# AlexandreGac/alphazero-chess

Hardware: AMD Instinct MI355X
Metric: MCTS sims/sec at 800 sims/move, 20x256 net; self-play games/hr at 1/2/4/8 GPU (higher is better)
Workload: dtype f32

## Files before the change

alphazero-chess_amd/azchess/_lib.py:

```python
import ctypes as C
import os

import numpy as np

_HERE = os.path.dirname(os.path.abspath(__file__))
LIB_PATH = os.environ.get("AZ_LIB") or os.path.join(_HERE, "libaz.so")
CSRC = os.path.join(os.path.dirname(_HERE), "csrc")

ACTION_SPACE = 4096
MAX_MOVES = 256
ONGOING, DRAW, WHITE_WINS, BLACK_WINS, ILLEGAL = 0, 1, 2, 3, -1
DTYPE_F32, DTYPE_BF16, DTYPE_FP8 = 0, 1, 2
EVAL_NET, EVAL_SYNTHETIC, EVAL_CALLBACK = 0, 1, 2
PACKED_KINDS = ("conv_w", "conv_b", "in_pk32", "wino_w", "wino16_w", "wino16_us", "w8", "w8s", "b8", "head",
                "head_frag", "head_frag32")


class AzPos(C.Structure):
    _fields_ = [("bb", C.c_uint64 * 8), ("turn", C.c_uint8), ("castling", C.c_uint8), ("ep", C.c_uint8),
                ("flags", C.c_uint8), ("halfmoves", C.c_uint16), ("fullmoves", C.c_uint16),
                ("rep_key", C.c_uint64)]


POS_DTYPE = np.dtype({
# ... 51 lines not shown
ALLREDUCE_FN = C.CFUNCTYPE(C.c_int, C.c_void_p, C.POINTER(C.c_float), C.c_size_t)

P = C.POINTER
SIGNATURES = [
    ("az_last_error", C.c_char_p, []),
    ("az_version", C.c_int, []),
    ("az_device_count", C.c_int, [P(C.c_int)]),
    ("az_device_synchronize", C.c_int, [C.c_int]),
    ("az_pos_startpos", C.c_int, [P(AzPos)]),
    ("az_pos_from_fen", C.c_int, [C.c_char_p, P(AzPos)]),
    ("az_pos_to_fen", C.c_int, [P(AzPos), C.c_char_p, C.c_int]),
    ("az_pos_fen_key", C.c_uint64, [P(AzPos)]),
    ("az_pos_legal_indices", C.c_int, [P(AzPos), P(C.c_int32), C.c_int]),
    ("az_pos_play_index", C.c_int, [P(AzPos), C.c_int32, P(AzPos)]),
    ("az_move_to_index", C.c_int, [C.c_int, C.c_int, C.c_int]),
    ("az_pos_outcome", C.c_int, [P(AzPos)]),
    ("az_pos_encode", C.c_int, [P(AzPos), P(C.c_float)]),
    ("az_game_create", C.c_int, [P(C.c_void_p)]),
    ("az_game_clone", C.c_int, [C.c_void_p, P(C.c_void_p)]),
    ("az_game_destroy", C.c_int, [C.c_void_p]),
    ("az_game_position", C.c_int, [C.c_void_p, P(AzPos)]),
    ("az_game_history", C.c_int, [C.c_void_p, P(C.c_int32), C.c_int]),
    ("az_game_play", C.c_int, [C.c_void_p, C.c_int32]),
    ("az_net_num_params", C.c_size_t, [C.c_int, C.c_int]),
    ("az_net_create", C.c_int, [P(AzNetDesc), P(C.c_float), C.c_size_t, C.c_int, P(C.c_void_p)]),
    ("az_net_destroy", C.c_int, [C.c_void_p]),
    ("az_net_tower_kernel", C.c_int, [C.c_void_p, C.c_char_p, C.c_int]),
    ("az_net_wino_streamed_points", C.c_int, [C.c_void_p]),
    ("az_net_wino_accumulators", C.c_int, [C.c_void_p]),
    ("az_net_wino_v_rows", C.c_int, [C.c_void_p]),
    ("az_wino_vrows_layout", C.c_int, [C.c_void_p] * 5),
    ("az_net_wino_boards", C.c_int, [C.c_void_p]),
    ("az_wino_boards_layout", C.c_int, [C.c_void_p] * 6),
    ("az_wino16_pack", C.c_int, [P(C.c_float), C.c_int, C.c_int, P(C.c_uint16), C.c_size_t, P(C.c_float)]),
    ("az_wino16_pack_rows", C.c_int, [P(C.c_float), C.c_int, P(C.c_uint16), C.c_size_t, P(C.c_float)]),
    ("az_net_load_mpk",C.c_int, [C.c_char_p, C.c_int, C.c_int, P(C.c_float), C.c_size_t]),
    ("az_net_save_mpk", C.c_int, [C.c_char_p, C.c_int, C.c_int, P(C.c_float), C.c_size_t]),
    ("az_net_forward", C.c_int, [C.c_void_p, P(C.c_float), C.c_int, P(C.c_float), P(C.c_float)]),
    ("az_net_forward_device", C.c_int, [C.c_void_p, C.c_void_p, C.c_int, C.c_void_p, C.c_void_p, C.c_void_p]),
    ("az_net_update_device", C.c_int, [C.c_void_p, C.c_void_p, C.c_size_t, C.c_void_p]),
    ("az_net_update", C.c_int, [C.c_void_p, P(C.c_float), C.c_size_t]),
    ("az_net_update_from_trainer", C.c_int, [C.c_void_p, C.c_void_p]),
    ("az_net_generation", C.c_int64, [C.c_void_p]),
    ("az_net_get_weights", C.c_int, [C.c_void_p, P(C.c_float), C.c_size_t]),
    ("az_net_packed_read", C.c_int, [C.c_void_p, C.c_int, C.c_int, C.c_void_p, C.c_size_t]),
    ("az_search_default_cfg", C.c_int, [P(AzSearchCfg)]),
    ("az_search_create", C.c_int, [C.c_void_p, P(AzSearchCfg), C.c_int, P(C.c_void_p)]),
    ("az_search_destroy", C.c_int, [C.c_void_p]),
    ("az_search_set_evaluator", C.c_int, [C.c_void_p, C.c_void_p, C.c_void_p]),
    ("az_search_set_roots", C.c_int, [C.c_void_p, P(C.c_int32), P(C.c_int32), P(C.c_int32), P(C.c_int32),
                                      C.c_int]),
    ("az_search_set_roots_from", C.c_int, [C.c_void_p, P(AzPos), P(C.c_int32), P(C.c_int32), P(C.c_int32),
                                           P(C.c_int32), C.c_int]),
    ("az_search_run", C.c_int, [C.c_void_p, P(C.c_float), P(C.c_uint32), P(C.c_int32)]),
    ("az_search_read_roots", C.c_int, [C.c_void_p, P(C.c_float), P(C.c_uint32), P(C.c_int32)]),
    ("az_search_advance", C.c_int, [C.c_void_p, P(C.c_int32), C.c_int, P(C.c_int32)]),
    ("az_selfplay_reset", C.c_int, [C.c_void_p]),
    ("az_selfplay_step", C.c_int, [C.c_void_p, P(C.c_int), P(C.c_int)]),
    ("az_selfplay_run_sims", C.c_int, [C.c_void_p, C.c_int, P(C.c_int), P(C.c_int), P(C.c_int)]),
    ("az_selfplay_drain", C.c_int, [C.c_void_p, P(AzEpisodeStep), C.c_int]),
    ("az_selfplay_adopt_net", C.c_int, [C.c_void_p]),
    ("az_search_adopt_net", C.c_int, [C.c_void_p, C.c_int]),
    ("az_selfplay_inflight", C.c_int, [C.c_void_p, P(C.c_int32), P(C.c_int32), P(C.c_int32), P(C.c_int32),
                                       P(C.c_int32), C.c_int]),
    ("az_search_stats_get", C.c_int, [C.c_void_p, P(AzSearchStats)]),
    ("az_search_persistent", C.c_int, [C.c_void_p]),
# ... 130 lines not shown
```

alphazero-chess_amd/azchess/agent.py:

```python
import ctypes as C
import os

import numpy as np

from . import _lib as L
from .parameters import NUM_FILTERS, NUM_RES_BLOCKS, SEED


def num_params(blocks, filters):
    return int(L.lib.az_net_num_params(int(blocks), int(filters)))


def param_shapes(blocks, filters):
    F = filters
    out = [("input_conv.weight", (F, 19, 3, 3), 19 * 9), ("input_conv.bias", (F,), 19 * 9),
           ("input_bn", (4, F), None)]
    for b in range(blocks):
        for k in (1, 2):
            out += [("res_blocks.%d.conv%d.weight" % (b, k), (F, F, 3, 3), F * 9),
                    ("res_blocks.%d.conv%d.bias" % (b, k), (F,), F * 9),
                    ("res_blocks.%d.bn%d" % (b, k), (4, F), None)]
    out += [("policy_conv_1.weight", (32, F, 1, 1), F), ("policy_conv_1.bias", (32,), F), ("policy_bn", (4, 32), None),
            ("policy_conv_2.weight", (64, 32, 1, 1), 32), ("policy_conv_2.bias", (64,), 32),
            ("value_conv.weight", (8, F, 1, 1), F), ("value_conv.bias", (8,), F), ("value_bn", (4, 8), None),
# ... 113 lines not shown
    @property
    def winograd(self):
        return "Winograd" in self.tower_kernel

    def __del__(self):
        try:
            L.lib.az_net_destroy(self._h)
        except Exception:
            pass

    def save_file(self, path):
        save_mpk(path, self.weights, self.blocks, self.filters)

    def forward(self, x):
        x = np.ascontiguousarray(x, np.float32).reshape(-1, 19 * 64)
        n = x.shape[0]
        pol = np.zeros((n, 4096), np.float32)
        val = np.zeros(n, np.float32)
        L.check(L.lib.az_net_forward(self._h, L.fptr(x), n, L.fptr(pol), L.fptr(val)))
        return pol, val


def wino_vrows_layout():
    t = dict(write=np.empty((16, 64, 4), np.int32), read=np.empty((2, 4, 4, 64), np.int32),
             act=np.empty((16, 64, 4), np.int32), item=np.empty((2, 8, 4), np.int32), dims=np.empty(4, np.int32))
    L.check(L.lib.az_wino_vrows_layout(*(t[k].ctypes.data_as(C.c_void_p) for k in ("write", "read", "act", "item", "dims"))))
    return t


def wino_boards_layout():
    t = dict(item=np.empty((8, 8, 2), np.int32), act=np.empty((2, 2), np.int32), out=np.empty((8, 64, 2, 4), np.int32),
             vbuf=np.empty((2, 2), np.int32), zero=np.empty(64, np.int32), dims=np.empty(8, np.int32))
    L.check(L.lib.az_wino_boards_layout(*(t[k].ctypes.data_as(C.c_void_p) for k in ("item", "act", "out", "vbuf", "zero", "dims"))))
    return t


def mx8_quantize(x):
    x = np.ascontiguousarray(x, np.float32)
    if x.size % 32:
        raise ValueError("mx8_quantize: %d values are not whole blocks of 32" % x.size)
    codes = np.empty(x.shape, np.uint8)
    scales = np.empty(x.size // 32, np.uint8)
    u8 = lambda a: a.ctypes.data_as(L.P(C.c_uint8))
    L.check(L.lib.az_mx8_quantize(L.fptr(x), x.size // 32, u8(codes), u8(scales)))
    return codes, scales


def mx8_conv_probe(filters, act_codes, act_scales, w_codes, w_scales, bias, residual=None, device=0):
    F = int(filters)
    a = np.ascontiguousarray(act_codes, np.uint8)
    n = a.size // (64 * F)
    s = np.ascontiguousarray(act_scales, np.uint8)
    wc, wsc = np.ascontiguousarray(w_codes, np.uint8), np.ascontiguousarray(w_scales, np.uint8)
    b = np.ascontiguousarray(bias, np.float32)
    if a.size != n * 64 * F or s.size != n * 64 * F // 32 or wc.size != F * F * 9 or wsc.size != F * 9 * F // 32 or b.size != F:
        raise ValueError("mx8_conv_probe: operand shapes do not match filters = %d" % F)
    r = None if residual is None else np.ascontiguousarray(residual, np.uint16)
    if r is not None and r.size != a.size:
        raise ValueError("mx8_conv_probe: residual shape")
    out = dict(acc=np.empty((n, 64, F), np.float32), codes=np.empty((n, 64, F), np.uint8),
               scales=np.empty((n, 64, F // 32), np.uint8))
    if r is not None:
        out["bf16"] = np.empty((n, 64, F), np.uint16)
    u8 = lambda x: x.ctypes.data_as(L.P(C.c_uint8))
    u16 = lambda x: None if x is None else x.ctypes.data_as(L.P(C.c_uint16))
    L.check(L.lib.az_mx8_conv_probe(int(device), F, n, u8(a), u8(s), u8(wc), u8(wsc), u16(r), L.fptr(b), L.fptr(out["acc"]),
# ... 3 lines not shown
```

alphazero-chess_amd/csrc/tower.hip:

```cpp
#include <math.h>
#include <stdio.h>
#include <stdlib.h>
#include <string.h>

#include "az_internal.h"
#include "search_dev.h"
#include "wino.h"

#include "tower_dev.h"

namespace azi {

template <int F, bool SEARCH>
__device__ __forceinline__ void tower_board(const __bf16* __restrict__ planes, const TowerArgs& ta, int row0, int nb,
                                            float* __restrict__ pol_out, float* __restrict__ val_out,
                                            const SearchOut& so, int tid) {
    constexpr int BPB = TowerCfg<F>::BPB, WB = TowerCfg<F>::WB, BPW = BPB / WB, NCO = TowerCfg<F>::NCO;
    constexpr int NCW = F / (16 * NCO);
    constexpr int NT = NCW * WB * 64;
    constexpr int RSF = F / 8 + 2, RSI = 32 / 8 + 2;
    constexpr int XSZ = BPB * 64 * RSF;
    constexpr int ZN = 16 + F / 8;
    constexpr int HSZ0 = (HeadsScratch<HeadsCfg<F>::NB, NT>::FLOATS * 4 + 15) / 16;
    constexpr int HSZ = ((XSZ > HSZ0 ? XSZ : HSZ0) + 15) / 16 * 16;
// ... 491 lines not shown
                                        : n * 1024 + wino_toff<F>(0, i * XS + rx);
                    wring[i][rx][n] = __builtin_bit_cast(f32x4, __builtin_amdgcn_raw_buffer_load_b128(r, voff + off, 0, 0));
                }
    }
    for (int b = 0; b < ta.blocks; b++) {
        const unsigned wb3 = b + 1 < ta.blocks ? ta.wwbytes[2 * b + 2] : 0u;
        const __amdgpu_buffer_rsrc_t r1 = t32_rsrc(ta.ww[2 * b], ta.wwbytes[2 * b]);
        const __amdgpu_buffer_rsrc_t r2 = t32_rsrc(ta.ww[2 * b + 1], ta.wwbytes[2 * b + 1]);
        const __amdgpu_buffer_rsrc_t r3 = t32_rsrc(b + 1 < ta.blocks ? ta.ww[2 * b + 2] : ta.ww[2 * b + 1], wb3);
        constexpr bool PRE = F == 256 || F == 64;
        conv_wino<F, false, H16, SP, ROWS, VROWS>(ldsb, vbase, r1, r2, ta.b[1 + 2 * b], ta.wus[2 * b], wring, xres, w, lane, PRE && b > 0, PRE, 0, flag,
                            2 * b + 1, tr ? tr + 3 + 64 * b : nullptr);
        conv_wino<F, true, H16, SP, ROWS, VROWS>(ldsb, vbase, r2, r3, ta.b[2 + 2 * b], ta.wus[2 * b + 1], wring, xres, w, lane, PRE, PRE && b + 1 < ta.blocks,
                           F == 64 ? 1 : 0, flag, 2 * b + 2, tr ? tr + 35 + 64 * b : nullptr);
    }
    heads_group<F, RSF, 1, NT, SEARCH, true, H16>(ldsb, reinterpret_cast<float*>(V), 0, 1, row0, tid, ta.head_frag32, ta.head,
                                             pol_out, val_out, so, tr);
    wino_stamp(tr, 3 + 64 * 20);
}

template <int F, bool SEARCH, bool H16, int SP = 16, bool ROWS = false, bool VROWS = false>
__global__ void __launch_bounds__(WinoCfg<F>::NWV * 64)
tower32w_kernel(const float* __restrict__ planes, TowerArgs ta, const int* __restrict__ count_ptr, int rows,
                float* __restrict__ pol_out, float* __restrict__ val_out, SearchOut so) {
    const int count = count_ptr ? min(load_fresh(count_ptr), rows) : rows;
    if ((int)blockIdx.x >= count) return;
    tower32w_board<F, SEARCH, H16, SP, ROWS, VROWS>(planes, ta, blockIdx.x, pol_out, val_out, so, threadIdx.x);
}

typedef unsigned int u32v4 __attribute__((__vector_size__(16)));
constexpr int WINO_B2_HS = (HeadsScratch<1, 512, heads_npart(512, true)>::FLOATS * 4 + 15) / 16;
constexpr int WINO_B2_AUX = ((WINO_B2_HS > 64 * 10 ? WINO_B2_HS : 64 * 10) + 15) / 16 * 16;
constexpr int WINO_B2_ZN = 16 + 256 / 4;
constexpr int WINO_B2_LDS = (WINO_B2_VBYTES / 16 + WINO_B2_AUX + WINO_B2_ZN + 1) * 16;
constexpr int WINO_B2_OVL = 0;
static_assert(WINO_B2_OVL % 256 == 0 && WINO_B2_OVL + WINO_B2_ACT <= WINO_B2_VBYTES, "the ACT overlay lies inside V");
__device__ __forceinline__ void b2_stores_done() { asm volatile("s_waitcnt vmcnt(0)" ::: "memory"); }

template <bool RESID>
__device__ __forceinline__ void conv_wino_b2(char* __restrict__ ldsv, const __amdgpu_buffer_rsrc_t rW,
                                             const __amdgpu_buffer_rsrc_t rN, const __amdgpu_buffer_rsrc_t rA,
                                             const float* __restrict__ bias, float unscale,
                                             f32x4 (&wr)[WINO_B2_PF][2][2], int w, int lane, bool pre_in, bool pre_out,
                                             int* flag, int seq, unsigned long long* tr = nullptr) {
    constexpr int HIN = RESID ? 1 : 0, HOUT = 1 - HIN;
    f32x4 acc[2][8][2];
    wino_stamp(tr, 0);
    wino_core_b2(ldsv, rW, rN, rA, HIN, wr, w, lane, pre_in, acc, tr);
    wino_stamp(tr, 10);
    const int ln = vgpr_index(lane);
    const int co0 = w * 32 + (ln >> 4) * 4;
    auto out_addr = [&](int n, int a, int b) { return wino_b2_out(w, ln, n, 2 * a + b); };
    f32x4 xres[2][4];
    auto xload = [&](int k) {
        if constexpr (RESID) {
#pragma unroll
            for (int q = 0; q < 4; q++)
                xres[k & 1][q] = __builtin_bit_cast(f32x4, __builtin_amdgcn_raw_buffer_load_b128(
                                                               rA, wino_b2_act(k >> 1, 0) + out_addr(k & 1, q >> 1, q & 1), 0, 0));
        }
    };
    xload(0);
    xload(1);
    (void)xres;
#pragma unroll
    for (int nb = 0; nb < 2; nb++)
#pragma unroll
        for (int n = 0; n < 2; n++) {
            f32x4 y[4];
            wino_rows_out(acc[nb], bias, unscale, co0, n, y);
            f32x4 o[4];
#pragma unroll
            for (int q = 0; q < 4; q++) {
                o[q] = y[q];
                if constexpr (RESID) o[q] += xres[n][q];
            }
            if (2 * nb + n + 2 < 4) xload(2 * nb + n + 2);
#pragma unroll
            for (int q = 0; q < 4; q++) {
                f32x4 v = o[q];
#pragma unroll
                for (int r = 0; r < 4; r++) v[r] = relu_nan<true>(v[r]);
                __builtin_amdgcn_raw_buffer_store_b128(__builtin_bit_cast(u32v4, v), rA,
                                                       wino_b2_act(nb, HOUT) + out_addr(n, q >> 1, q & 1), 0, 0);
            }
        }
    wino_stamp(tr, 11);
    b2_stores_done();
    if (pre_out && w < 4) {
        if (w == 0) __hip_atomic_store(flag, seq, __ATOMIC_RELEASE, __HIP_MEMORY_SCOPE_WORKGROUP);
        else
            while (__hip_atomic_load(flag, __ATOMIC_ACQUIRE, __HIP_MEMORY_SCOPE_WORKGROUP) != seq)
                __builtin_amdgcn_s_sleep(1);
        wino_b2_items<4>(ldsv, rA, HOUT, 0, 0, w, lane);
    }
    __syncthreads();
}

template <bool SEARCH>
__device__ __forceinline__ void tower32w_boards2(const float* __restrict__ planes, const TowerArgs& ta, int row0, int nbv,
                                                 char* __restrict__ act, float* __restrict__ pol_out,
                                                 float* __restrict__ val_out, const SearchOut& so, int tid) {
    constexpr int F = 256, NT = 512, NN = 2, RSF = F / 4 + 2, RSI = 32 / 4 + 2, PF = WINO_B2_PF;
    constexpr int VSZ = WINO_B2_VBYTES / 16, AUX = WINO_B2_AUX, ZN = WINO_B2_ZN;
    static_assert(64 * RSF <= VSZ && 64 * RSF * 16 == WINO_B2_ACT, "one board's ACT overlays V");
    static_assert(64 * RSI <= AUX, "input planes must fit in AUX");
    static_assert((VSZ + AUX) * 16 % 256 == 0, "conv32_in_packed ORs the zero row's offset into the low byte");
    static_assert(WINO_B2_LDS <= 163840, "LDS of a CU");
    __shared__ __attribute__((aligned(16))) uint4 lds[VSZ + AUX + ZN + 1];
    const int lane = tid & 63;
    const int w = __builtin_amdgcn_readfirstlane(tid >> 6);
    char* ldsb = reinterpret_cast<char*>(lds);
    char* actl = ldsb + WINO_B2_OVL;
    uint4* A = lds + VSZ;
    const int zero_off = (VSZ + AUX) * 16;
    int* flag = reinterpret_cast<int*>(lds + VSZ + AUX + ZN);
    const __amdgpu_buffer_rsrc_t rA = t32_rsrc(reinterpret_cast<const uint4*>(act), WINO_B2_WG);
    unsigned long long* tr = nullptr;
#ifdef AZ_TOWER_TRACE
    tr = tt_slot(w);
#endif
    wino_stamp(tr, 0);
    for (int c = tid; c < ZN + 1; c += NT) lds[VSZ + AUX + c] = make_uint4(0, 0, 0, 0);
#pragma unroll 1
    for (int nb = 0; nb < 2; nb++) {
        stage_planes_f32<1, RSI, NT>(A, planes, so, row0 + nb, nb < nbv ? 1 : 0, tid);
        __syncthreads();
        if (nb == 0) wino_stamp(tr, 1);
        {
            f32x4 wr[T32_PF][NN];
            const __amdgpu_buffer_rsrc_t r0 = t32_rsrc(ta.w0pk, ta.w0pk_bytes);
            const int voff = ((w * NN) * 64 + lane) * 16;
#pragma unroll
            for (int i = 0; i < T32_PF; i++)
#pragma unroll
                for (int n = 0; n < NN; n++)
                    wr[i][n] = __builtin_bit_cast(f32x4, __builtin_amdgcn_raw_buffer_load_b128(
                                                             r0, voff + n * 1024 + i * (F / 16) * 1024, 0, 0));
            conv32_in_packed<F, RSI, RSF, NN>(ldsb, actl, VSZ * 16, zero_off, r0, ta.b[0], wr, w, lane);
        }
        for (int i = tid; i < 64 * 64; i += NT) {
            const int o = ((i >> 6) * RSF + (i & 63)) * 16;
// ... 276 lines not shown
    for (int sched = 0; sched < 2; sched++)
        for (int wave = 0; wave < 8; wave++)
            for (int it = 0; it < 4; it++) {
                const int nw = sched ? 8 : 4;
                item[(sched * 8 + wave) * 4 + it] = wave < nw && it < WINO_VR_ITEMS / nw ? wino_vr_item(wave, it, nw) : -1;
            }
    dims[0] = WINO_VR_PLANE; dims[1] = WINO_VR_BYTES; dims[2] = WINO_VR_R16; dims[3] = 4;
    return 0;
}

extern "C" int az_wino_boards_layout(int* item, int* act, int* out, int* vbuf, int* zero, int* dims) {
    using namespace azi;
    if (!item || !act || !out || !vbuf || !zero || !dims) return fail("null argument");
    for (int w = 0; w < 8; w++)
        for (int k = 0; k < 8; k++) {
            item[(w * 8 + k) * 2] = k < wino_b2_item_count(w) ? wino_b2_item_board(w, k) : -1;
            item[(w * 8 + k) * 2 + 1] = k < wino_b2_item_count(w) ? wino_b2_item_q(w, k) : -1;
        }
    for (int nb = 0; nb < 2; nb++)
        for (int b = 0; b < 2; b++) {
            act[nb * 2 + b] = wino_b2_act(nb, b);
            vbuf[nb * 2 + b] = wino_b2_v(nb, b);
        }
    for (int w = 0; w < 8; w++)
        for (int lane = 0; lane < 64; lane++)
            for (int n = 0; n < 2; n++)
                for (int q = 0; q < 4; q++) out[((w * 64 + lane) * 2 + n) * 4 + q] = wino_b2_out(w, lane, n, q);
    for (int k = 0; k < 64; k++) zero[k] = wino_vr_zero(k);
    dims[0] = WINO_B2_ACT; dims[1] = WINO_B2_WG; dims[2] = WINO_VR_BYTES; dims[3] = WINO_B2_OVL; dims[4] = WINO_B2_ACT;
    dims[5] = WINO_B2_VBYTES; dims[6] = WINO_B2_AUX * 16; dims[7] = WINO_B2_LDS;
    return 0;
}

#ifdef AZ_TOWER_TRACE
extern "C" int az_tower_trace_read(unsigned long long* out, size_t n) {
    const size_t cap = sizeof(azi::az_tower_trace_buf) / sizeof(unsigned long long);
    if (hipDeviceSynchronize() != hipSuccess) return -1;
    return hipMemcpyFromSymbol(out, HIP_SYMBOL(azi::az_tower_trace_buf), (n < cap ? n : cap) * 8) == hipSuccess ? 0 : -1;
}
#endif
```

alphazero-chess_amd/csrc/wino.h:

```cpp
#pragma once
#include "az_internal.h"

namespace azi {

typedef __attribute__((ext_vector_type(4))) float f32x4;
typedef __attribute__((ext_vector_type(2))) float f32x2;

#define AZ_PK2(name, mods)                                                                    \
    __device__ __forceinline__ f32x2 name(f32x2 a, f32x2 b) {                                 \
        f32x2 r;                                                                              \
        asm("v_pk_add_f32 %0, %1, %2 " mods : "=v"(r) : "v"(a), "v"(b));                      \
        return r;                                                                             \
    }
#define AZ_PK3(name, mods)                                                                    \
    __device__ __forceinline__ f32x2 name(f32x2 a, f32x2 m, f32x2 b) {                        \
        f32x2 r;                                                                              \
        asm("v_pk_fma_f32 %0, %1, %2, %3 " mods : "=v"(r) : "v"(a), "v"(m), "v"(b));          \
        return r;                                                                             \
    }
AZ_PK2(pk_add, "")
AZ_PK2(pk_sub, "neg_lo:[0,1] neg_hi:[0,1]")
AZ_PK2(pk_rowa, "op_sel_hi:[1,0] neg_lo:[0,1]")
AZ_PK2(pk_rowb, "op_sel:[1,0] neg_lo:[0,1] neg_hi:[0,1]")
AZ_PK2(pk_negx_add, "neg_lo:[1,1]")
// ... 45 lines not shown

typedef __attribute__((ext_vector_type(8))) _Float16 f16x8;
template <int F> __device__ __forceinline__ int wino16_voff(int w, int lane) {
    return (2 * WinoCfg<F>::NN * w * 64 + lane) * 16;
}

constexpr int WINO_XF_FULL = 0, WINO_XF_NEG1 = 1, WINO_XF_COLS = 2;

constexpr int WINO_VR_PLANE = 10240, WINO_VR_BYTES = 2 * WINO_VR_PLANE, WINO_VR_ITEMS = 16;
constexpr int WINO_VR_R16 = (256 / 4 + 2) * 16;
__host__ __device__ constexpr int wino_vr_lo(int a) { return (a ^ 32) + WINO_VR_PLANE; }
__host__ __device__ constexpr int wino_vr_lo_if(int lo, int a) { return lo ? wino_vr_lo(a) : a; }
__host__ __device__ constexpr int wino_vr_item(int wave, int it, int nw) { return wave + nw * it; }
__host__ __device__ constexpr int wino_vr_item_row(int q) { return 1 + (q >> 1); }
__host__ __device__ constexpr int wino_vr_wuni(int q) {
    const int r = wino_vr_item_row(q), rp = (r >> 1) & 1;
    return ((r & 1) * 5 + (r >> 1)) * 256 + (((q & 1) ^ rp) * 2) * 64;
}
__host__ __device__ constexpr int wino_vr_wlane(int lane) {
    return wino_vr_lo_if(lane & 1, ((lane >> 3) & 1) * 64 + (lane >> 4) * 16) + ((lane & 7) >> 1) * 4;
}
__host__ __device__ constexpr int wino_vr_wpoint(int b) { return b * 2560; }
__host__ __device__ constexpr int wino_vr_write(int q, int lane, int b) { return wino_vr_wuni(q) + wino_vr_wlane(lane) + wino_vr_wpoint(b); }
__host__ __device__ constexpr int wino_vr_rlane(int lane, int i2) {
    const int h = lane >> 4, tr = (lane & 15) >> 2, tc = lane & 3;
    const int a0 = tr * 256 + (4 * (h ^ (2 * (tr & 1))) + tc) * 16;
    return i2 ? (a0 ^ 128) + 256 : a0;
}
__host__ __device__ constexpr int wino_vr_rimm(int i, int b) { return (2 * b + (i & 1)) * 5 * 256; }
__host__ __device__ constexpr int wino_vr_read(int i, int b, int lane) { return wino_vr_rlane(lane, i >> 1) + wino_vr_rimm(i, b); }
__host__ __device__ constexpr int wino_vr_zero(int k) {
    return (k >> 4) * WINO_VR_BYTES + ((k >> 3) & 1) * WINO_VR_PLANE + (k & 1 ? (2 * ((k >> 1) & 3) + 1) * 5 + 4 : 2 * ((k >> 1) & 3) * 5) * 256;
}
__host__ __device__ constexpr int wino_vr_alane(int lane) { return (lane >> 4) * (2 * WINO_VR_R16) + (lane & 15) * 4; }
__host__ __device__ constexpr int wino_vr_acol(int tc, int j) {
    return j == 0 ? (tc > 0 ? -WINO_VR_R16 : 3 * WINO_VR_R16) : j == 1 ? 0 : j == 2 ? WINO_VR_R16
                                                                  : (tc < 3 ? 2 * WINO_VR_R16 : -2 * WINO_VR_R16);
}
__host__ __device__ constexpr int wino_vr_auni(int q) { return (wino_vr_item_row(q) - 1) * 8 * WINO_VR_R16 + (q & 1) * 64; }
__host__ __device__ constexpr int wino_vr_act(int q, int lane, int j) { return wino_vr_auni(q) + wino_vr_alane(lane) + wino_vr_acol(lane >> 4, j); }
template <int F> struct WinoXf {
    static constexpr int NWV = WinoCfg<F>::NWV, CH = WinoCfg<F>::CH, RS = F / 4 + 2;
    static constexpr int VBYTES = CH * 1024, XST = CH * 64, IT = CH * 16 / (NWV * 64);
    static constexpr int R16 = RS * 16, ROW = 8 * R16;
    typedef f32x2 Patch[IT][4][2];
    char* ldsb;
    int vbase, w, lane, tty, ttx;
    __device__ __forceinline__ WinoXf(char* l, int vb, int w_, int lane_)
        : ldsb(l), vbase(vb), w(w_), lane(lane_), tty(w_ & 3), ttx(lane_ >> 4) {}
    __device__ __forceinline__ int tchan(int it, int g) const { return 16 * ((w >> 2) + g + it * (NWV / 4)) + (lane & 15); }
    __device__ __forceinline__ int vwr(int tch) const {
        return (tch >> 2) * 256 + (((4 * tty + ttx) ^ (2 * ((tch >> 2) & 3))) * 16) + (tch & 3) * 4;
    }
    __device__ __forceinline__ void load(int c, Patch& d, int g = 0) const {
        const int tl = vgpr_index(ttx);
        const int pc1 = tl * (2 * R16) + (lane & 15) * 4;
        const int pd0 = tl > 0 ? -R16 : 3 * R16, pd3 = tl < 3 ? 2 * R16 : -2 * R16;
#pragma unroll
        for (int it = 0; it < IT; it++) {
            const int b1 = pc1 + (2 * tty - 1) * ROW + (c * CH + tchan(it, g) - (lane & 15)) * 4;
            const int cb[4] = {b1 + pd0, b1, b1 + R16, b1 + pd3};
#pragma unroll
            for (int j = 0; j < 4; j++) {
                const char* p = ldsb + cb[j];
                d[it][j][0] = f32x2{*reinterpret_cast<const float*>(p), *reinterpret_cast<const float*>(p + ROW)};
                d[it][j][1] = f32x2{*reinterpret_cast<const float*>(p + 2 * ROW), *reinterpret_cast<const float*>(p + 3 * ROW)};
            }
        }
    }
    static __device__ __forceinline__ void xform(const f32x2 (&d)[4][2], f32x2 m, f32x2 (&v)[4][2]) {
        f32x2 A[4], B[4];
#pragma unroll
// ... 613 lines not shown

constexpr int WINO_B2_ACT = 64 * WINO_VR_R16;
constexpr int WINO_B2_BOARD = 2 * WINO_B2_ACT;
constexpr int WINO_B2_WG = 2 * WINO_B2_BOARD;
constexpr int WINO_B2_VBYTES = 4 * WINO_VR_BYTES;
#ifndef AZ_WINO_B2_PF
#define AZ_WINO_B2_PF 3
#endif
constexpr int WINO_B2_PF = AZ_WINO_B2_PF;
static_assert(12 % WINO_B2_PF == 0 && WINO_B2_PF >= 2, "the ring's slots must be compile-time");
__host__ __device__ constexpr int wino_b2_act(int nb, int hbuf) { return nb * WINO_B2_BOARD + hbuf * WINO_B2_ACT; }
__host__ __device__ constexpr int wino_b2_v(int nb, int buf) { return (2 * nb + buf) * WINO_VR_BYTES; }
__host__ __device__ constexpr int wino_b2_out(int w, int lane, int n, int q) {
    const int l16 = lane & 15, ty = l16 >> 2, tx = l16 & 3;
    return ((2 * ty + (q >> 1)) * 8 + 2 * tx + (q & 1)) * WINO_VR_R16 + (w * 32 + (lane >> 4) * 4 + n * 16) * 4;
}
#ifndef AZ_WINO_B2_XE
#define AZ_WINO_B2_XE 6
#endif
constexpr int WINO_B2_XE = AZ_WINO_B2_XE, WINO_B2_XL = 8 - WINO_B2_XE;
static_assert(WINO_B2_XE >= 4 && WINO_B2_XE <= 8, "waves 0-3 take at least their share, at most everything");
__host__ __device__ constexpr int wino_b2_item_count(int w) { return w < 4 ? WINO_B2_XE : WINO_B2_XL; }
__host__ __device__ constexpr int wino_b2_item_g(int w, int k) { return w < 4 ? w + 4 * k : 4 * WINO_B2_XE + (w - 4) + 4 * k; }
__host__ __device__ constexpr int wino_b2_item_board(int w, int k) { return wino_b2_item_g(w, k) >> 4; }
__host__ __device__ constexpr int wino_b2_item_q(int w, int k) { return wino_b2_item_g(w, k) & 15; }

__device__ __forceinline__ void wino_b2_load(const __amdgpu_buffer_rsrc_t rA, int aoff, int c, int q, float (&e)[4], int ln) {
    const int tl = ln >> 4;
    const int p = wino_vr_alane(ln) + wino_vr_auni(q) + c * 128 + aoff;
#pragma unroll
    for (int j = 0; j < 4; j++)
        e[j] = __builtin_bit_cast(float, __builtin_amdgcn_raw_buffer_load_b32(rA, p + wino_vr_acol(tl, j), 0, 0));
}
template <int NW>
__device__ __forceinline__ void wino_b2_items(char* __restrict__ ldsv, const __amdgpu_buffer_rsrc_t rA, int hbuf, int c,
                                              int buf, int w, int lane) {
    constexpr int NI = WINO_VR_ITEMS / NW;
    const int ln = vgpr_index(lane);
    float e[2][NI][4];
#pragma unroll
    for (int nb = 0; nb < 2; nb++)
#pragma unroll
        for (int i = 0; i < NI; i++) wino_b2_load(rA, wino_b2_act(nb, hbuf), c, wino_vr_item(w, i, NW), e[nb][i], ln);
#pragma unroll
    for (int nb = 0; nb < 2; nb++) {
        const WinoXf<256> xf(ldsv, wino_b2_v(nb, 0), w, lane);
#pragma unroll
        for (int i = 0; i < NI; i++) xf.vr_store(buf, wino_vr_item(w, i, NW), e[nb][i], ln);
    }
}

__device__ __forceinline__ void wino_rows_out(const f32x4 (&acc)[8][2], const float* __restrict__ bias, float unscale,
                                              int co0, int n, f32x4 (&y)[4]) {
    const f32x2 us = f32x2{unscale, unscale};
    {
        const f32x4 bb = *reinterpret_cast<const f32x4*>(bias + co0 + n * 16);
#pragma unroll
        for (int p = 0; p < 2; p++) {
            f32x2 s0[4], s1[4];
#pragma unroll
            for (int j = 0; j < 4; j++) {
                s0[j] = p ? f32x2{acc[j][n][2], acc[j][n][3]} : f32x2{acc[j][n][0], acc[j][n][1]};
                s1[j] = p ? f32x2{acc[4 + j][n][2], acc[4 + j][n][3]} : f32x2{acc[4 + j][n][0], acc[4 + j][n][1]};
            }
            const f32x2 br = p ? f32x2{bb[2], bb[3]} : f32x2{bb[0], bb[1]};
            const f32x2 q0 = pkc_fma(pk_add(pk_add(s0[0], s0[1]), s0[2]), us, br);
            const f32x2 q1 = pkc_fma(pk_sub(pk_sub(s0[1], s0[2]), s0[3]), us, br);
            const f32x2 q2 = pkc_fma(pk_add(pk_add(s1[0], s1[1]), s1[2]), us, br);
            const f32x2 q3 = pkc_fma(pk_sub(pk_sub(s1[1], s1[2]), s1[3]), us, br);
            y[0][2 * p] = q0.x; y[0][2 * p + 1] = q0.y;
            y[1][2 * p] = q1.x; y[1][2 * p + 1] = q1.y;
            y[2][2 * p] = q2.x; y[2][2 * p + 1] = q2.y;
            y[3][2 * p] = q3.x; y[3][2 * p + 1] = q3.y;
        }
    }
}

__device__ __forceinline__ void wino_core_b2(char* __restrict__ ldsv, const __amdgpu_buffer_rsrc_t rW,
                                             const __amdgpu_buffer_rsrc_t rN, const __amdgpu_buffer_rsrc_t rA, int hin,
                                             f32x4 (&wr)[WINO_B2_PF][2][2], int w, int lane, bool pre,
                                             f32x4 (&acc)[2][8][2], unsigned long long* tr = nullptr) {
    constexpr int F = 256, CF = F / 16, NN = 2, PF = WINO_B2_PF, NCHUNK = 8, SPX = 12, STEPB = CF * 2 * 1024;
    const int vr0 = wino_vr_rlane(lane, 0), vr1 = wino_vr_rlane(lane, 1);
#pragma unroll
    for (int nb = 0; nb < 2; nb++)
#pragma unroll
        for (int x = 0; x < 8; x++)
#pragma unroll
            for (int n = 0; n < NN; n++) {
                f32x2 z0, z1;
                asm volatile("v_mov_b64 %0, 0" : "=v"(z0));
                asm volatile("v_mov_b64 %0, 0" : "=v"(z1));
                acc[nb][x][n] = f32x4{z0.x, z0.y, z1.x, z1.y};
            }
    const int voff = wino16_voff<F>(w, lane);
    if (!pre) {
        wino_b2_items<8>(ldsv, rA, hin, 0, 0, w, lane);
        __syncthreads();
    }
    wino_stamp(tr, 1);
#pragma unroll 1
    for (int c = 0; c < NCHUNK; c++) {
        const bool more = c + 1 < NCHUNK;
        f16x8 bw[2][2][2];
        float en[4];
        auto bread = [&](int nb, int st) {
            const char* vb = ldsv + wino_b2_v(nb, c & 1);
#pragma unroll
            for (int s = st % 3 == 0 ? 0 : 1; s < 2; s++) {
                const int n = 4 * (st / 3) + st % 3 + s;
                const int vl = (n % 4) >> 1 ? vr1 : vr0;
                const char* p = vb + wino_vr_rimm(n % 4, n / 4);
                bw[nb][n % 2][0] = *reinterpret_cast<const f16x8*>(p + vl);
                bw[nb][n % 2][1] = *reinterpret_cast<const f16x8*>(p + wino_vr_lo(vl));
            }
        };
        bread(0, 0);
        bread(1, 0);
#pragma unroll
        for (int st = 0; st < SPX; st++) {
            const int b = st / 3;
            if (more) {
                if (st >= 1 && st <= wino_b2_item_count(w)) {
                    const WinoXf<F> xf(ldsv, wino_b2_v(wino_b2_item_board(w, st - 1), 0), w, lane);
                    xf.vr_store((c + 1) & 1, wino_b2_item_q(w, st - 1), en, vgpr_index(lane));
                }
                if (st < wino_b2_item_count(w))
                    wino_b2_load(rA, wino_b2_act(wino_b2_item_board(w, st), hin), c + 1, wino_b2_item_q(w, st), en, vgpr_index(lane));
            }
#pragma unroll
            for (int nb = 0; nb < 2; nb++) {
                __builtin_amdgcn_sched_barrier(0);
#pragma unroll
                for (int term = 0; term < 3; term++)
#pragma unroll
                    for (int pt = 0; pt < 2; pt++)
#pragma unroll
                        for (int n = 0; n < NN; n++) {
                            const f16x8 av = __builtin_bit_cast(f16x8, wr[st % PF][term == 2 ? 1 : 0][n]);
                            const f16x8 bv = bw[nb][(4 * b + st % 3 + pt) % 2][term == 1 ? 1 : 0];
                            acc[nb][4 * pt + b][n] = __builtin_amdgcn_mfma_f32_16x16x32_f16(av, bv, acc[nb][4 * pt + b][n], 0, 0, 0);
                        }
                __builtin_amdgcn_sched_barrier(0);
                if (nb == 1) {
                    const bool nxt = st + PF >= SPX && !more;
                    const int tn = c * SPX + st + PF;
                    const int to = nxt ? tn - NCHUNK * SPX : tn;
#pragma unroll
                    for (int pl = 0; pl < 2; pl++)
#pragma unroll
                        for (int n = 0; n < NN; n++)
                            wr[st % PF][pl][n] = __builtin_bit_cast(
                                f32x4, __builtin_amdgcn_raw_buffer_load_b128(nxt ? rN : rW, voff + (2 * n + pl) * 1024,
                                                                             to * STEPB, 0));
                }
                if (st + 1 < SPX) bread(nb, st + 1);
            }
            if (st == 4) wino_stamp(tr, 20 + c);
        }
        wino_stamp(tr, 12 + c);
        if (more) __syncthreads();
        wino_stamp(tr, 2 + c);
    }
}

}
```

include/az.h:

```cpp
#ifndef AZ_H
#define AZ_H
#include <stddef.h>
#include <stdint.h>

#ifdef __cplusplus
extern "C" {
#endif

#define AZ_ACTION_SPACE 4096
#define AZ_PLANES 19
#define AZ_MAX_MOVES 256

enum { AZ_ONGOING = 0, AZ_DRAW = 1, AZ_WHITE_WINS = 2, AZ_BLACK_WINS = 3, AZ_ILLEGAL = -1 };

typedef struct az_pos {
    uint64_t bb[8];
    uint8_t turn, castling, ep, flags;
    uint16_t halfmoves, fullmoves;
    uint64_t rep_key;
} az_pos;

const char* az_last_error(void);
int az_version(void);
int az_device_count(int* n);
int az_device_synchronize(int device);

int az_pos_startpos(az_pos* out);
int az_pos_from_fen(const char* fen, az_pos* out);
int az_pos_to_fen(const az_pos* p, char* buf, int cap);
uint64_t az_pos_fen_key(const az_pos* p);
int az_pos_legal_indices(const az_pos* p, int32_t* out, int cap);
int az_pos_play_index(const az_pos* p, int32_t index, az_pos* child);
int az_move_to_index(int from, int to, int turn);
int az_pos_outcome(const az_pos* p);
int az_pos_encode(const az_pos* p, float* out);

typedef struct az_game az_game;
int az_game_create(az_game** out);
int az_game_clone(const az_game* g, az_game** out);
int az_game_destroy(az_game* g);
int az_game_position(const az_game* g, az_pos* out);
int az_game_history(const az_game* g, int32_t* moves, int cap);
int az_game_play(az_game* g, int32_t index);

enum { AZ_DTYPE_F32 = 0, AZ_DTYPE_BF16 = 1, AZ_DTYPE_FP8 = 2 };
typedef struct { int blocks, filters, dtype; } az_net_desc;
typedef struct az_net az_net;
size_t az_net_num_params(int blocks, int filters);
int az_net_create(const az_net_desc* desc, const float* weights, size_t n, int device, az_net** out);
int az_net_destroy(az_net* net);
int az_net_tower_kernel(az_net* net, char* out, int cap);
int az_net_wino_streamed_points(az_net* net);
int az_net_wino_accumulators(az_net* net);
int az_net_wino_v_rows(az_net* net);
int az_net_wino_boards(az_net* net);
int az_wino_boards_layout(int* item, int* act, int* out, int* vbuf, int* zero, int* dims);
int az_wino_vrows_layout(int* write, int* read, int* act, int* item, int* dims);
int az_net_load_mpk(const char* path, int blocks, int filters, float* out, size_t n);
int az_net_save_mpk(const char* path, int blocks, int filters, const float* w, size_t n);
int az_net_forward(az_net* net, const float* planes, int n, float* policy, float* value);
int az_net_forward_device(az_net* net, const float* d_planes, int n, float* d_policy, float* d_value,
                          void* stream);
int az_net_update_device(az_net* net, const float* d_weights, size_t n, void* stream);
int az_net_update(az_net* net, const float* weights, size_t n);
int64_t az_net_generation(az_net* net);
int az_net_get_weights(az_net* net, float* out, size_t n);
enum {
    AZ_PACKED_CONV_W = 0, AZ_PACKED_CONV_B = 1, AZ_PACKED_IN_PK32 = 2, AZ_PACKED_WINO_W = 3, AZ_PACKED_WINO16_W = 4,
    AZ_PACKED_WINO16_US = 5, AZ_PACKED_W8 = 6, AZ_PACKED_W8S = 7, AZ_PACKED_B8 = 8, AZ_PACKED_HEAD = 9,
    AZ_PACKED_HEAD_FRAG = 10, AZ_PACKED_HEAD_FRAG32 = 11, AZ_PACKED_KINDS = 12
};
int az_net_packed_read(az_net* net, int kind, int index, void* out, size_t cap);

enum { AZ_EVAL_NET = 0, AZ_EVAL_SYNTHETIC = 1, AZ_EVAL_CALLBACK = 2 };
typedef int (*az_eval_fn)(void* ctx, const az_pos* positions, int n, float* policy, float* value);
typedef struct {
    int games;
    int sims;
    float c_puct;
    float dir_alpha;
    float dir_eps;
    int temp_moves;
    int noise;
    uint64_t seed;
    int evaluator;
    int continuous;
    int record_evals;
    int eval_log_cap;
    int cache_capacity;
// ... 176 lines not shown
```

Measured before the change: 212,400.

## Stage block-boundary outputs in an LDS slice to feed the next pre-transform

At the residual-block boundary, wave 0 also writes its activated outputs into a new LDS slice. The next block's Winograd pre-transform then reads from that slice instead of global memory, so it no longer waits on a vmcnt(0) drain before starting. The bias is hoisted out of the loop, the residual prefetch depth becomes configurable, and an optional s_setprio knob is added (off by default). A layout query is exported for tests. This costs extra LDS per workgroup, which may lower occupancy.

```diff
diff --git a/alphazero-chess_amd/azchess/_lib.py b/alphazero-chess_amd/azchess/_lib.py
--- a/alphazero-chess_amd/azchess/_lib.py
+++ b/alphazero-chess_amd/azchess/_lib.py
@@ -107,6 +107,7 @@
     ("az_wino_vrows_layout", C.c_int, [C.c_void_p] * 5),
     ("az_net_wino_boards", C.c_int, [C.c_void_p]),
     ("az_wino_boards_layout", C.c_int, [C.c_void_p] * 6),
+    ("az_wino_boundary_layout", C.c_int, [C.c_void_p] * 5),
     ("az_wino16_pack", C.c_int, [P(C.c_float), C.c_int, C.c_int, P(C.c_uint16), C.c_size_t, P(C.c_float)]),
     ("az_wino16_pack_rows", C.c_int, [P(C.c_float), C.c_int, P(C.c_uint16), C.c_size_t, P(C.c_float)]),
     ("az_net_load_mpk",C.c_int, [C.c_char_p, C.c_int, C.c_int, P(C.c_float), C.c_size_t]),
diff --git a/alphazero-chess_amd/azchess/agent.py b/alphazero-chess_amd/azchess/agent.py
--- a/alphazero-chess_amd/azchess/agent.py
+++ b/alphazero-chess_amd/azchess/agent.py
@@ -169,6 +169,13 @@
     t = dict(item=np.empty((8, 8, 2), np.int32), act=np.empty((2, 2), np.int32), out=np.empty((8, 64, 2, 4), np.int32),
              vbuf=np.empty((2, 2), np.int32), zero=np.empty(64, np.int32), dims=np.empty(8, np.int32))
     L.check(L.lib.az_wino_boards_layout(*(t[k].ctypes.data_as(C.c_void_p) for k in ("item", "act", "out", "vbuf", "zero", "dims"))))
+    return t
+
+
+def wino_boundary_layout():
+    t = dict(sl_out=np.empty((64, 2, 4), np.int32), sl_act=np.empty((16, 64, 4), np.int32), item=np.empty((8, 4), np.int32),
+             region=np.empty((10, 4), np.int32), dims=np.empty(8, np.int32))
+    L.check(L.lib.az_wino_boundary_layout(*(t[k].ctypes.data_as(C.c_void_p) for k in ("sl_out", "sl_act", "item", "region", "dims"))))
     return t
 
 
diff --git a/alphazero-chess_amd/csrc/tower.hip b/alphazero-chess_amd/csrc/tower.hip
--- a/alphazero-chess_amd/csrc/tower.hip
+++ b/alphazero-chess_amd/csrc/tower.hip
@@ -547,7 +547,9 @@
 constexpr int WINO_B2_HS = (HeadsScratch<1, 512, heads_npart(512, true)>::FLOATS * 4 + 15) / 16;
 constexpr int WINO_B2_AUX = ((WINO_B2_HS > 64 * 10 ? WINO_B2_HS : 64 * 10) + 15) / 16 * 16;
 constexpr int WINO_B2_ZN = 16 + 256 / 4;
-constexpr int WINO_B2_LDS = (WINO_B2_VBYTES / 16 + WINO_B2_AUX + WINO_B2_ZN + 1) * 16;
+constexpr int WINO_B2_SLN = WINO_B2_SL_BYTES / 16;
+constexpr int WINO_B2_SL_OFF = (WINO_B2_VBYTES / 16 + WINO_B2_AUX + WINO_B2_ZN + 1) * 16;
+constexpr int WINO_B2_LDS = WINO_B2_SL_OFF + WINO_B2_SL_BYTES;
 constexpr int WINO_B2_OVL = 0;
 static_assert(WINO_B2_OVL % 256 == 0 && WINO_B2_OVL + WINO_B2_ACT <= WINO_B2_VBYTES, "the ACT overlay lies inside V");
 __device__ __forceinline__ void b2_stores_done() { asm volatile("s_waitcnt vmcnt(0)" ::: "memory"); }
@@ -566,31 +568,38 @@
     const int ln = vgpr_index(lane);
     const int co0 = w * 32 + (ln >> 4) * 4;
     auto out_addr = [&](int n, int a, int b) { return wino_b2_out(w, ln, n, 2 * a + b); };
-    f32x4 xres[2][4];
+    f32x4 bb[2];
+    if constexpr (AZ_WINO_B2_BIAS2) {
+#pragma unroll
+        for (int n = 0; n < 2; n++) bb[n] = *reinterpret_cast<const f32x4*>(bias + co0 + n * 16);
+    }
+    constexpr int RA = AZ_WINO_B2_RA;
+    f32x4 xres[RA][4];
     auto xload = [&](int k) {
         if constexpr (RESID) {
 #pragma unroll
             for (int q = 0; q < 4; q++)
-                xres[k & 1][q] = __builtin_bit_cast(f32x4, __builtin_amdgcn_raw_buffer_load_b128(
-                                                               rA, wino_b2_act(k >> 1, 0) + out_addr(k & 1, q >> 1, q & 1), 0, 0));
+                xres[k % RA][q] = __builtin_bit_cast(f32x4, __builtin_amdgcn_raw_buffer_load_b128(
+                                                                rA, wino_b2_act(k >> 1, 0) + out_addr(k & 1, q >> 1, q & 1), 0, 0));
         }
     };
-    xload(0);
-    xload(1);
+#pragma unroll
+    for (int k = 0; k < RA; k++) xload(k);
     (void)xres;
 #pragma unroll
     for (int nb = 0; nb < 2; nb++)
 #pragma unroll
         for (int n = 0; n < 2; n++) {
             f32x4 y[4];
-            wino_rows_out(acc[nb], bias, unscale, co0, n, y);
+            if constexpr (!AZ_WINO_B2_BIAS2) bb[n] = *reinterpret_cast<const f32x4*>(bias + co0 + n * 16);
+            wino_rows_out(acc[nb], bb[n], unscale, n, y);
             f32x4 o[4];
 #pragma unroll
             for (int q = 0; q < 4; q++) {
                 o[q] = y[q];
-                if constexpr (RESID) o[q] += xres[n][q];
-            }
-            if (2 * nb + n + 2 < 4) xload(2 * nb + n + 2);
+                if constexpr (RESID) o[q] += xres[(2 * nb + n) % RA][q];
+            }
+            if (2 * nb + n + RA < 4) xload(2 * nb + n + RA);
 #pragma unroll
             for (int q = 0; q < 4; q++) {
                 f32x4 v = o[q];
@@ -598,17 +607,32 @@
                 for (int r = 0; r < 4; r++) v[r] = relu_nan<true>(v[r]);
                 __builtin_amdgcn_raw_buffer_store_b128(__builtin_bit_cast(u32v4, v), rA,
                                                        wino_b2_act(nb, HOUT) + out_addr(n, q >> 1, q & 1), 0, 0);
+                if constexpr (AZ_WINO_B2_SLICE)
+                    if (pre_out && w == 0)
+                        *reinterpret_cast<f32x4*>(ldsv + WINO_B2_SL_OFF + nb * WINO_B2_SL_BOARD + wino_b2_sl_out(ln, n, q)) = v;
             }
         }
     wino_stamp(tr, 11);
-    b2_stores_done();
-    if (pre_out && w < 4) {
-        if (w == 0) __hip_atomic_store(flag, seq, __ATOMIC_RELEASE, __HIP_MEMORY_SCOPE_WORKGROUP);
-        else
-            while (__hip_atomic_load(flag, __ATOMIC_ACQUIRE, __HIP_MEMORY_SCOPE_WORKGROUP) != seq)
-                __builtin_amdgcn_s_sleep(1);
-        wino_b2_items<4>(ldsv, rA, HOUT, 0, 0, w, lane);
-    }
+    if constexpr (AZ_WINO_B2_SLICE) {
+        if (pre_out && w < AZ_WINO_B2_SLW) {
+            if (w == 0) __hip_atomic_store(flag, seq, __ATOMIC_RELEASE, __HIP_MEMORY_SCOPE_WORKGROUP);
+            else
+                while (__hip_atomic_load(flag, __ATOMIC_ACQUIRE, __HIP_MEMORY_SCOPE_WORKGROUP) != seq)
+                    __builtin_amdgcn_s_sleep(1);
+            wino_b2_items_sl<AZ_WINO_B2_SLW>(ldsv, ldsv + WINO_B2_SL_OFF, w, lane);
+        }
+        b2_stores_done();
+    } else {
+        b2_stores_done();
+        if (pre_out && w < 4) {
+            if (w == 0) __hip_atomic_store(flag, seq, __ATOMIC_RELEASE, __HIP_MEMORY_SCOPE_WORKGROUP);
+            else
+                while (__hip_atomic_load(flag, __ATOMIC_ACQUIRE, __HIP_MEMORY_SCOPE_WORKGROUP) != seq)
+                    __builtin_amdgcn_s_sleep(1);
+            wino_b2_items<4>(ldsv, rA, HOUT, 0, 0, w, lane);
+        }
+    }
+    wino_stamp(tr, 28);
     __syncthreads();
 }
 
@@ -622,7 +646,8 @@
     static_assert(64 * RSI <= AUX, "input planes must fit in AUX");
     static_assert((VSZ + AUX) * 16 % 256 == 0, "conv32_in_packed ORs the zero row's offset into the low byte");
     static_assert(WINO_B2_LDS <= 163840, "LDS of a CU");
-    __shared__ __attribute__((aligned(16))) uint4 lds[VSZ + AUX + ZN + 1];
+    static_assert((VSZ + AUX + ZN + 1) * 16 == WINO_B2_SL_OFF, "the slice lies behind the flag");
+    __shared__ __attribute__((aligned(16))) uint4 lds[VSZ + AUX + ZN + 1 + WINO_B2_SLN];
     const int lane = tid & 63;
     const int w = __builtin_amdgcn_readfirstlane(tid >> 6);
     char* ldsb = reinterpret_cast<char*>(lds);
@@ -965,6 +990,39 @@
     return 0;
 }
 
+extern "C" int az_wino_boundary_layout(int* sl_out, int* sl_act, int* item, int* region, int* dims) {
+    using namespace azi;
+    if (!sl_out || !sl_act || !item || !region || !dims) return fail("null argument");
+    for (int lane = 0; lane < 64; lane++)
+        for (int n = 0; n < 2; n++)
+            for (int q = 0; q < 4; q++) sl_out[(lane * 2 + n) * 4 + q] = wino_b2_sl_out(lane, n, q);
+    for (int q = 0; q < WINO_VR_ITEMS; q++)
+        for (int lane = 0; lane < 64; lane++)
+            for (int j = 0; j < 4; j++) sl_act[(q * 64 + lane) * 4 + j] = wino_b2_sl_act(q, lane, j);
+    constexpr int NW = AZ_WINO_B2_SLICE ? AZ_WINO_B2_SLW : 4;
+    for (int wave = 0; wave < 8; wave++)
+        for (int it = 0; it < 4; it++)
+            item[wave * 4 + it] = wave < NW && it < WINO_VR_ITEMS / NW ? wino_vr_item(wave, it, NW) : -1;
+    enum { IN = 1, C06 = 2, C7 = 4, EPI = 8, PRE = 16, HEADS = 32 };
+    int r = 0;
+    auto add = [&](int off, int bytes, int live, int kind) {
+        region[r * 4] = off; region[r * 4 + 1] = bytes; region[r * 4 + 2] = live; region[r * 4 + 3] = kind;
+        r++;
+    };
+    for (int nb = 0; nb < 2; nb++) {
+        add(wino_b2_v(nb, 0), WINO_VR_BYTES, C06 | PRE, 0);
+        add(wino_b2_v(nb, 1), WINO_VR_BYTES, C06 | C7, 1);
+    }
+    add(WINO_B2_OVL, WINO_B2_ACT, IN | HEADS, 2);
+    add(WINO_B2_VBYTES, WINO_B2_AUX * 16, IN | HEADS, 3);
+    add(WINO_B2_VBYTES + WINO_B2_AUX * 16, WINO_B2_ZN * 16, IN, 4);
+    add(WINO_B2_VBYTES + (WINO_B2_AUX + WINO_B2_ZN) * 16, 16, C06 | C7 | EPI | PRE, 5);
+    for (int nb = 0; nb < 2; nb++) add(WINO_B2_SL_OFF + nb * WINO_B2_SL_BOARD, WINO_B2_SL_BOARD, EPI | PRE, 6);
+    dims[0] = WINO_B2_SL_OFF; dims[1] = WINO_B2_SL_BOARD; dims[2] = WINO_B2_SL_COL; dims[3] = WINO_B2_SL_ROW;
+    dims[4] = WINO_B2_LDS; dims[5] = NW; dims[6] = AZ_WINO_B2_SLICE ? 1 : 0; dims[7] = r;
+    return 0;
+}
+
 #ifdef AZ_TOWER_TRACE
 extern "C" int az_tower_trace_read(unsigned long long* out, size_t n) {
     const size_t cap = sizeof(azi::az_tower_trace_buf) / sizeof(unsigned long long);
diff --git a/alphazero-chess_amd/csrc/wino.h b/alphazero-chess_amd/csrc/wino.h
--- a/alphazero-chess_amd/csrc/wino.h
+++ b/alphazero-chess_amd/csrc/wino.h
@@ -101,12 +101,11 @@
 __host__ __device__ constexpr int wino_vr_zero(int k) {
     return (k >> 4) * WINO_VR_BYTES + ((k >> 3) & 1) * WINO_VR_PLANE + (k & 1 ? (2 * ((k >> 1) & 3) + 1) * 5 + 4 : 2 * ((k >> 1) & 3) * 5) * 256;
 }
-__host__ __device__ constexpr int wino_vr_alane(int lane) { return (lane >> 4) * (2 * WINO_VR_R16) + (lane & 15) * 4; }
-__host__ __device__ constexpr int wino_vr_acol(int tc, int j) {
-    return j == 0 ? (tc > 0 ? -WINO_VR_R16 : 3 * WINO_VR_R16) : j == 1 ? 0 : j == 2 ? WINO_VR_R16
-                                                                  : (tc < 3 ? 2 * WINO_VR_R16 : -2 * WINO_VR_R16);
-}
-__host__ __device__ constexpr int wino_vr_auni(int q) { return (wino_vr_item_row(q) - 1) * 8 * WINO_VR_R16 + (q & 1) * 64; }
+__host__ __device__ constexpr int wino_vr_alane(int lane, int cs = WINO_VR_R16) { return (lane >> 4) * (2 * cs) + (lane & 15) * 4; }
+__host__ __device__ constexpr int wino_vr_acol(int tc, int j, int cs = WINO_VR_R16) {
+    return j == 0 ? (tc > 0 ? -cs : 3 * cs) : j == 1 ? 0 : j == 2 ? cs : (tc < 3 ? 2 * cs : -2 * cs);
+}
+__host__ __device__ constexpr int wino_vr_auni(int q, int rs = 8 * WINO_VR_R16) { return (wino_vr_item_row(q) - 1) * rs + (q & 1) * 64; }
 __host__ __device__ constexpr int wino_vr_act(int q, int lane, int j) { return wino_vr_auni(q) + wino_vr_alane(lane) + wino_vr_acol(lane >> 4, j); }
 template <int F> struct WinoXf {
     static constexpr int NWV = WinoCfg<F>::NWV, CH = WinoCfg<F>::CH, RS = F / 4 + 2;
@@ -786,6 +785,53 @@
     for (int j = 0; j < 4; j++)
         e[j] = __builtin_bit_cast(float, __builtin_amdgcn_raw_buffer_load_b32(rA, p + wino_vr_acol(tl, j), 0, 0));
 }
+#ifndef AZ_WINO_B2_SLICE
+#define AZ_WINO_B2_SLICE 1
+#endif
+#ifndef AZ_WINO_B2_SLW
+#define AZ_WINO_B2_SLW 4
+#endif
+static_assert(AZ_WINO_B2_SLW == 4 || AZ_WINO_B2_SLW == 8, "the waves of the boundary's pre-transform");
+#ifndef AZ_WINO_B2_BIAS2
+#define AZ_WINO_B2_BIAS2 1
+#endif
+#ifndef AZ_WINO_B2_RA
+#define AZ_WINO_B2_RA 2
+#endif
+static_assert(AZ_WINO_B2_RA >= 1 && AZ_WINO_B2_RA <= 4, "fragments of residual in flight");
+#ifndef AZ_WINO_B2_PRIO7
+#define AZ_WINO_B2_PRIO7 0
+#endif
+static_assert(AZ_WINO_B2_PRIO7 >= 0 && AZ_WINO_B2_PRIO7 <= 12, "steps of a chunk");
+constexpr int WINO_B2_SL_COL = 160, WINO_B2_SL_ROW = 8 * WINO_B2_SL_COL + 16, WINO_B2_SL_BOARD = 8 * WINO_B2_SL_ROW;
+constexpr int WINO_B2_SL_BYTES = AZ_WINO_B2_SLICE ? 2 * WINO_B2_SL_BOARD : 0;
+__host__ __device__ constexpr int wino_b2_sl_out(int lane, int n, int q) {
+    const int l16 = lane & 15, ty = l16 >> 2, tx = l16 & 3;
+    return (2 * ty + (q >> 1)) * WINO_B2_SL_ROW + (2 * tx + (q & 1)) * WINO_B2_SL_COL + ((lane >> 4) * 4 + n * 16) * 4;
+}
+__host__ __device__ constexpr int wino_b2_sl_act(int q, int lane, int j) {
+    return wino_vr_auni(q, WINO_B2_SL_ROW) + wino_vr_alane(lane, WINO_B2_SL_COL) + wino_vr_acol(lane >> 4, j, WINO_B2_SL_COL);
+}
+template <int NW>
+__device__ __forceinline__ void wino_b2_items_sl(char* __restrict__ ldsv, const char* __restrict__ sl, int w, int lane) {
+    constexpr int NI = WINO_VR_ITEMS / NW;
+    const int ln = vgpr_index(lane);
+    float e[2][NI][4];
+#pragma unroll
+    for (int nb = 0; nb < 2; nb++)
+#pragma unroll
+        for (int i = 0; i < NI; i++)
+#pragma unroll
+            for (int j = 0; j < 4; j++)
+                e[nb][i][j] = *reinterpret_cast<const float*>(sl + nb * WINO_B2_SL_BOARD + wino_b2_sl_act(wino_vr_item(w, i, NW), ln, j));
+#pragma unroll
+    for (int nb = 0; nb < 2; nb++) {
+        const WinoXf<256> xf(ldsv, wino_b2_v(nb, 0), w, lane);
+#pragma unroll
+        for (int i = 0; i < NI; i++) xf.vr_store(0, wino_vr_item(w, i, NW), e[nb][i], ln);
+    }
+}
+
 template <int NW>
 __device__ __forceinline__ void wino_b2_items(char* __restrict__ ldsv, const __amdgpu_buffer_rsrc_t rA, int hbuf, int c,
                                               int buf, int w, int lane) {
@@ -804,11 +850,9 @@
     }
 }
 
-__device__ __forceinline__ void wino_rows_out(const f32x4 (&acc)[8][2], const float* __restrict__ bias, float unscale,
-                                              int co0, int n, f32x4 (&y)[4]) {
+__device__ __forceinline__ void wino_rows_out(const f32x4 (&acc)[8][2], const f32x4 bb, float unscale, int n, f32x4 (&y)[4]) {
     const f32x2 us = f32x2{unscale, unscale};
     {
-        const f32x4 bb = *reinterpret_cast<const f32x4*>(bias + co0 + n * 16);
 #pragma unroll
         for (int p = 0; p < 2; p++) {
             f32x2 s0[4], s1[4];
@@ -874,6 +918,12 @@
 #pragma unroll
         for (int st = 0; st < SPX; st++) {
             const int b = st / 3;
+            if constexpr (AZ_WINO_B2_PRIO7 > 0) {
+                if (!more && w >= 4) {
+                    if (st == 0) __builtin_amdgcn_s_setprio(2);
+                    if (st == AZ_WINO_B2_PRIO7) __builtin_amdgcn_s_setprio(0);
+                }
+            }
             if (more) {
                 if (st >= 1 && st <= wino_b2_item_count(w)) {
                     const WinoXf<F> xf(ldsv, wino_b2_v(wino_b2_item_board(w, st - 1), 0), w, lane);
@@ -912,6 +962,9 @@
             }
             if (st == 4) wino_stamp(tr, 20 + c);
         }
+        if constexpr (AZ_WINO_B2_PRIO7 >= SPX) {
+            if (!more && w >= 4) __builtin_amdgcn_s_setprio(0);
+        }
         wino_stamp(tr, 12 + c);
         if (more) __syncthreads();
         wino_stamp(tr, 2 + c);
diff --git a/include/az.h b/include/az.h
--- a/include/az.h
+++ b/include/az.h
@@ -55,6 +55,7 @@
 int az_net_wino_v_rows(az_net* net);
 int az_net_wino_boards(az_net* net);
 int az_wino_boards_layout(int* item, int* act, int* out, int* vbuf, int* zero, int* dims);
+int az_wino_boundary_layout(int* sl_out, int* sl_act, int* item, int* region, int* dims);
 int az_wino_vrows_layout(int* write, int* read, int* act, int* item, int* dims);
 int az_net_load_mpk(const char* path, int blocks, int filters, float* out, size_t n);
 int az_net_save_mpk(const char* path, int blocks, int filters, const float* w, size_t n);
```

Measured after the change: 213,200, median of 6. About the same (+0.4%).
